# SmartBFT-Go/consensus

Hardware: NVIDIA H100
Metric: ECDSA-P256 verifies/sec at batch=64K (higher is better)
Workload: dtype u32 limbs (integer)

## Files before the change

### consensus_b200/csrc/inst_common.cuh

```cuda
#pragma once
#include "key_cache.cuh"
#include "keygroup.cuh"
#include "ops.h"

namespace sbv {

template <class C> struct Cfg;
template <> struct Cfg<P256> {
    static constexpr int COZ_MINB = 6, GPART_MINB = 6, KT_MINB = 6, COMB_MINB = 6;
    static constexpr bool KT_INL = true, COMB_INL = true;
};
template <> struct Cfg<P384> {
    static constexpr int COZ_MINB = 4, GPART_MINB = 3, KT_MINB = 4;
    static constexpr bool KT_INL = false;
};

template <class C>
cudaError_t op_gtable_init(uint32_t *gtab, cudaStream_t st) {
    const size_t entries = (size_t)C::GWINS << C::GW;
    k_gtable_init<C><<<(unsigned)((entries + 127) / 128), 128, 0, st>>>(gtab);
    return cudaGetLastError();
}

template <class C>
cudaError_t op_prep(uint32_t n, const uint8_t *r, const uint8_t *s, const uint8_t *dig, uint32_t dlen, uint32_t *uw, uint8_t *flags,
                    cudaStream_t st) {
    return launch_prep<C, 8>(n, r, s, dig, dlen, uw, flags, st);
}

template <class C>
cudaError_t op_group(uint32_t n, const uint8_t *qx, const uint8_t *qy, uint32_t seed, uint32_t hmask, uint32_t *htab, uint32_t *rep,
                     uint32_t *kcnt, uint32_t threshold, uint32_t max_keys, int32_t *keyid, uint32_t *keylist, uint32_t *counters,
                     cudaStream_t st) {
    const unsigned blocks = (n + 255) / 256;
    k_kg_insert<<<blocks, 256, 0, st>>>(n, KgXY<C>{qx, qy}, seed, hmask, htab, rep, kcnt);
    k_kg_assign<<<blocks, 256, 0, st>>>(n, rep, kcnt, threshold, max_keys, keyid, keylist, counters);
    return cudaGetLastError();
}

inline cudaError_t op_route(uint32_t n, const uint32_t *rep, const int32_t *keyid, int32_t *item_kid, uint32_t *klist, uint32_t *glist,
                            uint32_t *counters, cudaStream_t st) {
    k_kg_route<<<(n + 255) / 256, 256, 0, st>>>(n, rep, keyid, item_kid, klist, glist, counters);
    return cudaGetLastError();
}

template <class C>
cudaError_t op_gpart(uint32_t n, const uint32_t *uw, const uint32_t *gtab, uint32_t *gacc, cudaStream_t st) {
    constexpr int BLOCK = 64;
    k_gpart<C, BLOCK, Cfg<C>::GPART_MINB><<<(n + BLOCK - 1) / BLOCK, BLOCK, 0, st>>>(n, uw, reinterpret_cast<const uint4 *>(gtab), gacc);
    return cudaGetLastError();
}

template <class C>
cudaError_t op_coz(uint32_t n, const uint8_t *qx, const uint8_t *qy, const uint8_t *r, const uint32_t *uw, const uint8_t *flags,
                   const uint32_t *gtab, uint32_t *tscr, uint8_t *ok, const uint32_t *list, const uint32_t *count, cudaStream_t st) {
    constexpr int BLOCK = 64;
    const size_t smem = (size_t)7 * 2 * C::N * 4 * BLOCK;
    k_verify_coz<C, BLOCK, Cfg<C>::COZ_MINB><<<(n + BLOCK - 1) / BLOCK, BLOCK, smem, st>>>(
        n, qx, qy, r, uw, flags, reinterpret_cast<const uint4 *>(gtab), tscr, ok, list, count);
    return cudaGetLastError();
}

template <class C, int W>
cudaError_t op_kt_build(const uint32_t *nkeys_ptr, uint32_t cap, const uint32_t *keylist, const uint8_t *qx, const uint8_t *qy,
                        uint32_t *bases, uint32_t *hs, uint32_t *ztop, uint32_t *pref, uint32_t *ktab, uint8_t *keyflags, cudaStream_t st) {
    using KT = KeyTab<32 * C::N, W>;
    const unsigned kb = (cap + 63) / 64;
    const unsigned wb = (unsigned)(((size_t)cap * KT::NWIN + 63) / 64);
    k_kt_bases4<C, KT><<<(unsigned)(((size_t)cap * 4 + 127) / 128), 128, 0, st>>>(nkeys_ptr, cap, keylist, qx, qy, bases, keyflags);
    k_kt_fill<C, W><<<wb, 64, 0, st>>>(nkeys_ptr, cap, bases, keyflags, hs, ztop, ktab);
    k_kt_inv<C, KT><<<kb, 64, 0, st>>>(nkeys_ptr, cap, keyflags, ztop, pref);
    k_kt_final<C, KT><<<wb, 64, 0, st>>>(nkeys_ptr, cap, bases, keyflags, hs, ztop, ktab);
    return cudaGetLastError();
}

template <class C, int W>
cudaError_t op_kt_verify_grouped(uint32_t n, const int32_t *kidmap, const uint8_t *keyflags, const uint8_t *r, const uint32_t *uw, const uint8_t *flags,
                                 const uint32_t *gtab, const uint32_t *ktab, uint8_t *ok, const uint32_t *list, const uint32_t *count,
                                 const uint32_t *gacc, cudaStream_t st) {
    constexpr int BLOCK = 64;
    k_verify_kt<C, W, BLOCK, Cfg<C>::KT_MINB, false, Cfg<C>::KT_INL><<<(n + BLOCK - 1) / BLOCK, BLOCK, 0, st>>>(
        n, nullptr, kidmap, 0, keyflags, r, uw, flags, reinterpret_cast<const uint4 *>(gtab), reinterpret_cast<const uint4 *>(ktab), ok, list, count,
        gacc);
    return cudaGetLastError();
}

template <class C, int W>
cudaError_t op_kt_verify_registered(uint32_t n, const uint32_t *slot, const int32_t *slot2local, uint32_t n_slots, const uint8_t *keyflags,
                                    const uint8_t *r, const uint32_t *uw, const uint8_t *flags, const uint32_t *gtab, const uint32_t *ktab,
                                    uint8_t *ok, int warp, cudaStream_t st) {
    constexpr int BLOCK = 64;
    const uint4 *g4 = reinterpret_cast<const uint4 *>(gtab), *k4 = reinterpret_cast<const uint4 *>(ktab);
    if (warp)
        k_verify_kt_warp<C, W><<<(unsigned)(((size_t)n * 32 + 127) / 128), 128, 0, st>>>(n, slot, slot2local, n_slots, keyflags, r, uw, flags, g4, k4, ok);
    else
        k_verify_kt<C, W, BLOCK, Cfg<C>::KT_MINB, true, Cfg<C>::KT_INL><<<(n + BLOCK - 1) / BLOCK, BLOCK, 0, st>>>(
            n, slot, slot2local, n_slots, keyflags, r, uw, flags, g4, k4, ok, nullptr, nullptr, nullptr);
    return cudaGetLastError();
}

template <class C>
cudaError_t op_comb_build(const uint32_t *nkeys_ptr, uint32_t cap, const uint32_t *keylist, const uint8_t *qx, const uint8_t *qy,
                          uint32_t *bases, uint32_t *hs, uint32_t *ztop, uint32_t *pref, uint32_t *ktab, uint8_t *keyflags, cudaStream_t st) {
    using CT = CombTab<C>;
    const unsigned kb = (cap + 63) / 64;
    const unsigned cb = (unsigned)(((size_t)cap * CT::NCHAIN + 63) / 64);
    k_kt_bases4<C, CT><<<(unsigned)(((size_t)cap * 4 + 127) / 128), 128, 0, st>>>(nkeys_ptr, cap, keylist, qx, qy, bases, keyflags);
    k_comb_affine<C><<<kb, 64, 0, st>>>(nkeys_ptr, cap, keyflags, bases, pref);
    k_comb_fill<C><<<cb, 64, 0, st>>>(nkeys_ptr, cap, bases, keyflags, hs, ztop, ktab);
    k_kt_inv<C, CT><<<kb, 64, 0, st>>>(nkeys_ptr, cap, keyflags, ztop, pref);
    k_kt_final<C, CT><<<cb, 64, 0, st>>>(nkeys_ptr, cap, bases, keyflags, hs, ztop, ktab);
    return cudaGetLastError();
}

template <class C>
cudaError_t op_comb_verify(uint32_t n, const int32_t *kidmap, const uint8_t *keyflags, const uint8_t *r, const uint32_t *uw, const uint8_t *flags,
                           const uint32_t * , const uint32_t *ktab, uint8_t *ok, const uint32_t *list,
                           const uint32_t *count, const uint32_t *gacc, cudaStream_t st) {
    constexpr int BLOCK = 64;
    k_verify_comb<C, BLOCK, Cfg<C>::COMB_MINB, Cfg<C>::COMB_INL><<<(n + BLOCK - 1) / BLOCK, BLOCK, 0, st>>>(
        n, kidmap, keyflags, r, uw, flags, reinterpret_cast<const uint4 *>(ktab), ok, list, count, gacc);
    return cudaGetLastError();
}

template <class C>
cudaError_t op_kc_lookup(const uint32_t *nkeys_ptr, uint32_t kcap, const uint32_t *keylist, const uint8_t *qx, const uint8_t *qy, KcMap c, uint32_t tw4,
                         int32_t *keyid, uint32_t *lk, uint8_t *keyflags, uint32_t *ktab, cudaStream_t st) {
    k_kc_lookup<<<(unsigned)(((size_t)kcap * 32 + 127) / 128), 128, 0, st>>>(nkeys_ptr, kcap, keylist, KcXY<C>{qx, qy}, c, tw4, keyid, lk, keyflags,
                                                                            reinterpret_cast<uint4 *>(ktab));
    return cudaGetLastError();
}

template <class C>
cudaError_t op_kc_insert(uint32_t kcap, const uint32_t *lk, const uint8_t *qx, const uint8_t *qy, KcMap c, uint32_t tw4, const uint8_t *keyflags,
                         const uint32_t *ktab, cudaStream_t st) {
    k_kc_insert<<<(unsigned)(((size_t)kcap * 32 + 127) / 128), 128, 0, st>>>(kcap, lk, KcXY<C>{qx, qy}, c, tw4, keyflags,
                                                                            reinterpret_cast<const uint4 *>(ktab));
    return cudaGetLastError();
}

template <class C, class KT>
constexpr KtGeom kt_geom() {
    using KS = KtSizes<C, KT>;
    return KtGeom{KS::bases_words(1), KS::hs_words(1), KS::ztop_words(1), KS::ktab_words(1)};
}

}
```

### consensus_b200/csrc/keygroup.cuh

```cuda
#pragma once
#include "kernels.cuh"

namespace sbv {

constexpr uint32_t KG_EMPTY = 0xffffffffu;

SBV_DEV uint32_t kg_mix(uint32_t h, uint32_t w) {
    h = (h ^ w) * 0x9E3779B1u;
    h ^= h >> 15;
    return h * 0x85EBCA77u;
}
template <class C>
SBV_DEV uint32_t kg_hash(const uint8_t *__restrict__ qx_be, const uint8_t *__restrict__ qy_be, uint32_t i, uint32_t seed) {
    const uint32_t *x = reinterpret_cast<const uint32_t *>(qx_be + (size_t)i * C::BYTES);
    const uint32_t *y = reinterpret_cast<const uint32_t *>(qy_be + (size_t)i * C::BYTES);
    uint32_t h = seed;
#pragma unroll
    for (int k = 0; k < C::N; k++) {
        h = kg_mix(h, __ldg(x + k));
        h = kg_mix(h, __ldg(y + k));
    }
    return h ^ (h >> 16);
}
template <class C>
SBV_DEV bool kg_same_key(const uint8_t *__restrict__ qx_be, const uint8_t *__restrict__ qy_be, uint32_t i, uint32_t j) {
    const uint32_t *xi = reinterpret_cast<const uint32_t *>(qx_be + (size_t)i * C::BYTES);
    const uint32_t *xj = reinterpret_cast<const uint32_t *>(qx_be + (size_t)j * C::BYTES);
    const uint32_t *yi = reinterpret_cast<const uint32_t *>(qy_be + (size_t)i * C::BYTES);
    const uint32_t *yj = reinterpret_cast<const uint32_t *>(qy_be + (size_t)j * C::BYTES);
    uint32_t diff = 0;
#pragma unroll
    for (int k = 0; k < C::N; k++) diff |= (__ldg(xi + k) ^ __ldg(xj + k)) | (__ldg(yi + k) ^ __ldg(yj + k));
    return diff == 0;
}

template <class C>
struct KgXY {
    const uint8_t *qx_be, *qy_be;
    SBV_DEV uint32_t hash(uint32_t i, uint32_t seed) const { return kg_hash<C>(qx_be, qy_be, i, seed); }
    SBV_DEV bool same(uint32_t i, uint32_t j) const { return kg_same_key<C>(qx_be, qy_be, i, j); }
};
struct KgKey32 {
    const uint8_t *pub;
    SBV_DEV uint32_t hash(uint32_t i, uint32_t seed) const {
        const uint32_t *x = reinterpret_cast<const uint32_t *>(pub + (size_t)i * 32);
        uint32_t h = seed;
#pragma unroll
        for (int k = 0; k < 8; k += 2) {
            h = (h ^ __ldg(x + k)) * 0x9E3779B1u;
            h = (h ^ __ldg(x + k + 1)) * 0x85EBCA77u;
            h ^= h >> 15;
        }
        return h;
    }
    SBV_DEV bool same(uint32_t i, uint32_t j) const {
        const uint32_t *xi = reinterpret_cast<const uint32_t *>(pub + (size_t)i * 32);
        const uint32_t *xj = reinterpret_cast<const uint32_t *>(pub + (size_t)j * 32);
        uint32_t diff = 0;
#pragma unroll
        for (int k = 0; k < 8; k++) diff |= __ldg(xi + k) ^ __ldg(xj + k);
        return diff == 0;
    }
};

template <class KV>
__global__ void __launch_bounds__(256) k_kg_insert(uint32_t n, KV key, uint32_t seed, uint32_t hmask, uint32_t *__restrict__ htab,
                                                   uint32_t *__restrict__ rep, uint32_t *__restrict__ kcnt) {
    const uint32_t i = blockIdx.x * blockDim.x + threadIdx.x;
    if (i >= n) return;
    uint32_t h = key.hash(i, seed) & hmask;
    uint32_t r;
    for (;;) {
        uint32_t cur = htab[h];
        if (cur == KG_EMPTY) {
            cur = atomicCAS(htab + h, KG_EMPTY, i);
            if (cur == KG_EMPTY) { r = i; break; }
        }
        if (key.same(i, cur)) { r = cur; break; }
        h = (h + 1) & hmask;
    }
    rep[i] = r;
#if defined(__CUDA_ARCH__)
    const uint32_t peers = __match_any_sync(__activemask(), r);
    if ((threadIdx.x & 31) == (uint32_t)(__ffs((int)peers) - 1)) atomicAdd(kcnt + r, (uint32_t)__popc(peers));
#else
    atomicAdd(kcnt + r, 1u);
#endif
}

static __global__ void __launch_bounds__(256) k_kg_assign(uint32_t n, const uint32_t *__restrict__ rep, const uint32_t *__restrict__ kcnt,
                                                   uint32_t threshold, uint32_t max_keys, int32_t *__restrict__ keyid,
                                                   uint32_t *__restrict__ keylist, uint32_t *__restrict__ counters) {
    const uint32_t i = blockIdx.x * blockDim.x + threadIdx.x;
    if (i >= n) return;
    int32_t id = -1;
    if (rep[i] == i && kcnt[i] >= threshold) {
        const uint32_t k = atomicAdd(counters + 0, 1u);
        if (k < max_keys) { id = (int32_t)k; keylist[k] = i; }
    }
    keyid[i] = id;
}

static __global__ void __launch_bounds__(256) k_kg_route(uint32_t n, const uint32_t *__restrict__ rep, const int32_t *__restrict__ keyid,
                                                  int32_t *__restrict__ item_kid, uint32_t *__restrict__ klist, uint32_t *__restrict__ glist,
                                                  uint32_t *__restrict__ counters) {
    const uint32_t i = blockIdx.x * blockDim.x + threadIdx.x;
    const bool live = i < n;
    const int32_t kid = live ? keyid[rep[i]] : -1;
    if (live) item_kid[i] = kid;
#if defined(__CUDA_ARCH__)
    const uint32_t lane = threadIdx.x & 31;
    const uint32_t mk = __ballot_sync(0xffffffffu, live && kid >= 0), mg = __ballot_sync(0xffffffffu, live && kid < 0);
    uint32_t bk = 0, bg = 0;
    if (lane == 0) {
        if (mk) bk = atomicAdd(counters + 1, (uint32_t)__popc(mk));
        if (mg) bg = atomicAdd(counters + 2, (uint32_t)__popc(mg));
    }
    bk = __shfl_sync(0xffffffffu, bk, 0);
    bg = __shfl_sync(0xffffffffu, bg, 0);
    const uint32_t below = (1u << lane) - 1u;
    if (live && kid >= 0) klist[bk + __popc(mk & below)] = i;
    if (live && kid < 0) glist[bg + __popc(mg & below)] = i;
#else
    if (live && kid >= 0) klist[atomicAdd(counters + 1, 1u)] = i;
    if (live && kid < 0) glist[atomicAdd(counters + 2, 1u)] = i;
#endif
}


template <class C, class KT>
__global__ void __launch_bounds__(64) k_kt_bases(const uint32_t *__restrict__ nkeys_ptr, uint32_t cap, const uint32_t *__restrict__ keylist,
                                                 const uint8_t *__restrict__ qx_be, const uint8_t *__restrict__ qy_be,
                                                 uint32_t *__restrict__ bases, uint8_t *__restrict__ keyflags) {
    constexpr int N = C::N;
    const uint32_t k = blockIdx.x * blockDim.x + threadIdx.x;
    uint32_t nkeys = __ldg(nkeys_ptr);
    if (nkeys > cap) nkeys = cap;
    if (k >= nkeys) return;
    const uint32_t item = keylist ? keylist[k] : k;
    Jac<C> B;
    const bool good = load_key<C>(B.X, B.Y, qx_be, qy_be, item);
    keyflags[k] = good ? 1 : 0;
    if (!good) return;
    C::get_one(B.Z);
#pragma unroll 1
    for (int win = 0; win < KT::NBASE; win++) {
        if (win) {
#pragma unroll 1
            for (int d = 0; d < KT::STEP; d++) pt_double<C>(B);
        }
        uint32_t *o = bases + (size_t)win * 3 * N * cap + k;
#pragma unroll
        for (int i = 0; i < N; i++) { o[(size_t)i * cap] = B.X[i]; o[(size_t)(N + i) * cap] = B.Y[i]; o[(size_t)(2 * N + i) * cap] = B.Z[i]; }
    }
}

template <class C, class KT>
__global__ void __launch_bounds__(128) k_kt_bases4(const uint32_t *__restrict__ nkeys_ptr, uint32_t cap, const uint32_t *__restrict__ keylist,
                                                   const uint8_t *__restrict__ qx_be, const uint8_t *__restrict__ qy_be,
                                                   uint32_t *__restrict__ bases, uint8_t *__restrict__ keyflags) {
    constexpr int N = C::N;
    const uint32_t gt = blockIdx.x * blockDim.x + threadIdx.x;
    const uint32_t k = gt >> 2, role = gt & 3;
    uint32_t nkeys = __ldg(nkeys_ptr);
    if (nkeys > cap) nkeys = cap;
    if (k >= nkeys) return;
    const unsigned qbase = (threadIdx.x & 31) & ~3u, qmask = 0xFu << qbase;
    const uint32_t item = keylist ? keylist[k] : k;
    uint32_t X[N], Y[N], Z[N];
    const bool good = load_key<C>(X, Y, qx_be, qy_be, item);
    if (role == 0) keyflags[k] = good ? 1 : 0;
    if (!good) return;
    C::get_one(Z);
    auto bcast = [&](uint32_t (&v)[N], unsigned src) {
#pragma unroll
        for (int i = 0; i < N; i++) v[i] = __shfl_sync(qmask, v[i], qbase + src);
    };
#pragma unroll 1
    for (int win = 0; win < KT::NBASE; win++) {
        if (win) {
#pragma unroll 1
            for (int d = 0; d < KT::STEP; d++) {
                uint32_t s[N], a[N], b[N], r1[N], r2[N], r3[N], r4[N], t1[N], t2[N];
                C::fadd(s, Y, Y);
                mp_select<N>(a, role == 1 || role == 2, s, Z);
                mp_select<N>(b, role == 1, s, Z);
                C::fmul(r1, a, b);
                uint32_t bb[N];
                mp_copy<N>(bb, r1);
                bcast(bb, 1);
                C::fsub(t1, X, r1);
                C::fadd(t2, X, r1);
                mp_select<N>(a, role == 0, t1, X);
                mp_select<N>(a, role == 2, bb, a);
                mp_select<N>(b, role == 0, t2, bb);
                C::fmul(r2, a, b);
                uint32_t alpha[N], half[N], beta4[N];
                C::fadd(t1, r2, r2);
                C::fadd(alpha, t1, r2);
                C::fhalf(half, r2);
                C::fmul(r3, alpha, alpha);
                mp_copy<N>(beta4, r2);
                bcast(beta4, 1);
                bcast(half, 2);
                uint32_t x3[N], y3[N];
                C::fadd(t1, beta4, beta4);
                C::fsub(x3, r3, t1);
                C::fsub(t2, beta4, x3);
                C::fmul(r4, alpha, t2);
                C::fsub(y3, r4, half);
                mp_copy<N>(X, x3); bcast(X, 0);
                mp_copy<N>(Y, y3); bcast(Y, 0);
                mp_copy<N>(Z, r1); bcast(Z, 2);
            }
        }
        if (role == 0) {
            uint32_t *o = bases + (size_t)win * 3 * N * cap + k;
#pragma unroll
            for (int i = 0; i < N; i++) { o[(size_t)i * cap] = X[i]; o[(size_t)(N + i) * cap] = Y[i]; o[(size_t)(2 * N + i) * cap] = Z[i]; }
        }
    }
}

template <class C>
SBV_DEV void zaddu(uint32_t (&X1)[C::N], uint32_t (&Y1)[C::N], const uint32_t (&X2)[C::N], const uint32_t (&Y2)[C::N],
                   uint32_t (&X3)[C::N], uint32_t (&Y3)[C::N], uint32_t (&h)[C::N]) {
    constexpr int N = C::N;
    uint32_t c[N], w1[N], w2[N], dy[N], d[N], a1[N], t[N];
    C::fsub(h, X1, X2);
    C::fsqr(c, h);
    C::fmul(w1, X1, c);
    C::fmul(w2, X2, c);
    C::fsub(dy, Y1, Y2);
    C::fsqr(d, dy);
    C::fsub(t, w1, w2);
    C::fmul(a1, Y1, t);
    C::fsub(X3, d, w1);
    C::fsub(X3, X3, w2);
    C::fsub(t, w1, X3);
    C::fmul(Y3, dy, t);
    C::fsub(Y3, Y3, a1);
    mp_copy<N>(X1, w1);
    mp_copy<N>(Y1, a1);
}

template <class C, int W>
__global__ void __launch_bounds__(64) k_kt_fill(const uint32_t *__restrict__ nkeys_ptr, uint32_t cap, const uint32_t *__restrict__ bases,
                                                const uint8_t *__restrict__ keyflags, uint32_t *__restrict__ hs,
                                                uint32_t *__restrict__ ztop, uint32_t *__restrict__ ktab) {
    constexpr int N = C::N;
    using KT = KeyTab<32 * N, W>;
    const uint32_t t = blockIdx.x * blockDim.x + threadIdx.x;
    uint32_t nkeys = __ldg(nkeys_ptr);
    if (nkeys > cap) nkeys = cap;
    if (t >= nkeys * KT::NWIN) return;
    const uint32_t k = t % nkeys, win = t / nkeys;
    if (!keyflags[k]) return;
    uint32_t bx[N], by[N], bz[N];
    {
        const uint32_t *o = bases + (size_t)win * 3 * N * cap + k;
#pragma unroll
        for (int i = 0; i < N; i++) { bx[i] = o[(size_t)i * cap]; by[i] = o[(size_t)(N + i) * cap]; bz[i] = o[(size_t)(2 * N + i) * cap]; }
    }
    uint32_t *out = ktab + ((size_t)k * KT::NWIN + win) * KT::ENT * 2 * N;
#pragma unroll
    for (int i = 0; i < N; i++) { out[i] = bx[i]; out[N + i] = by[i]; }
    Jac<C> P;
    mp_copy<N>(P.X, bx); mp_copy<N>(P.Y, by); mp_copy<N>(P.Z, bz);
    uint32_t h[N], h2[N], h3[N];
    C::fadd(h, by, by);
    pt_double<C>(P);
    C::fsqr(h2, h);
    C::fmul(h3, h2, h);
    C::fmul(bx, bx, h2);
    C::fmul(by, by, h3);
    uint32_t zacc[N];
    mp_copy<N>(zacc, P.Z);
    {
        uint32_t *hp = hs + ((size_t)win * (KT::ENT - 1) + 0) * N * cap + k;
#pragma unroll
        for (int i = 0; i < N; i++) { out[2 * N + i] = P.X[i]; out[3 * N + i] = P.Y[i]; hp[(size_t)i * cap] = h[i]; }
    }
    uint32_t px[N], py[N];
    mp_copy<N>(px, P.X); mp_copy<N>(py, P.Y);
#pragma unroll 1
    for (int e = 3; e <= KT::ENT; e++) {
        uint32_t x3[N], y3[N];
        zaddu<C>(bx, by, px, py, x3, y3, h);
        C::fmul(zacc, zacc, h);
        mp_copy<N>(px, x3); mp_copy<N>(py, y3);
        uint32_t *hp = hs + ((size_t)win * (KT::ENT - 1) + (e - 2)) * N * cap + k;
        uint32_t *oe = out + (size_t)(e - 1) * 2 * N;
#pragma unroll
        for (int i = 0; i < N; i++) { oe[i] = px[i]; oe[N + i] = py[i]; hp[(size_t)i * cap] = h[i]; }
    }
    uint32_t *zp = ztop + (size_t)win * N * cap + k;
#pragma unroll
    for (int i = 0; i < N; i++) zp[(size_t)i * cap] = zacc[i];
}

template <class C, class KT>
__global__ void __launch_bounds__(64) k_kt_inv(const uint32_t *__restrict__ nkeys_ptr, uint32_t cap, const uint8_t *__restrict__ keyflags,
                                               uint32_t *__restrict__ ztop, uint32_t *__restrict__ pref) {
    constexpr int N = C::N;
    const uint32_t k = blockIdx.x * blockDim.x + threadIdx.x;
    uint32_t nkeys = __ldg(nkeys_ptr);
    if (nkeys > cap) nkeys = cap;
    if (k >= nkeys || !keyflags[k]) return;
    uint32_t run[N];
    C::get_one(run);
#pragma unroll 1
    for (int win = 0; win < KT::NCHAIN; win++) {
        uint32_t z[N];
        const uint32_t *zp = ztop + (size_t)win * N * cap + k;
        uint32_t *pp = pref + (size_t)win * N * cap + k;
#pragma unroll
        for (int i = 0; i < N; i++) { z[i] = zp[(size_t)i * cap]; pp[(size_t)i * cap] = run[i]; }
        C::fmul(run, run, z);
    }
    uint32_t inv[N];
    p_inv<C>(inv, run);
#pragma unroll 1
    for (int win = KT::NCHAIN - 1; win >= 0; win--) {
        uint32_t z[N], pv[N], zi[N];
        uint32_t *zp = ztop + (size_t)win * N * cap + k;
        const uint32_t *pp = pref + (size_t)win * N * cap + k;
#pragma unroll
        for (int i = 0; i < N; i++) { z[i] = zp[(size_t)i * cap]; pv[i] = pp[(size_t)i * cap]; }
        C::fmul(zi, inv, pv);
        C::fmul(inv, inv, z);
#pragma unroll
        for (int i = 0; i < N; i++) zp[(size_t)i * cap] = zi[i];
    }
}

template <class C, class KT>
__global__ void __launch_bounds__(64) k_kt_final(const uint32_t *__restrict__ nkeys_ptr, uint32_t cap, const uint32_t *__restrict__ bases,
                                                 const uint8_t *__restrict__ keyflags, const uint32_t *__restrict__ hs,
                                                 const uint32_t *__restrict__ ztop, uint32_t *__restrict__ ktab) {
    constexpr int N = C::N;
    const uint32_t t = blockIdx.x * blockDim.x + threadIdx.x;
    uint32_t nkeys = __ldg(nkeys_ptr);
    if (nkeys > cap) nkeys = cap;
    if (t >= nkeys * KT::NCHAIN) return;
    const uint32_t k = t % nkeys, win = t / nkeys;
    if (!keyflags[k]) return;
    uint32_t zi[N];
    {
        const uint32_t *zp = ztop + (size_t)win * N * cap + k;
#pragma unroll
        for (int i = 0; i < N; i++) zi[i] = zp[(size_t)i * cap];
    }
    uint32_t *out = ktab + ((size_t)k * KT::NCHAIN + win) * KT::ENT * 2 * N;
    uint32_t x[N], y[N], h[N];
    {
        const uint32_t *oe = out + (size_t)(KT::ENT - 1) * 2 * N;
#pragma unroll
        for (int i = 0; i < N; i++) { x[i] = oe[i]; y[i] = oe[N + i]; }
    }
#pragma unroll 1
    for (int e = KT::ENT; e >= 1; e--) {
        uint32_t nx[N], ny[N], nh[N];
        if (e >= 2) {
            const uint32_t *on = out + (size_t)(e - 2) * 2 * N;
            const uint32_t *hp = hs + ((size_t)win * (KT::ENT - 1) + (e - 2)) * N * cap + k;
#pragma unroll
            for (int i = 0; i < N; i++) { nx[i] = on[i]; ny[i] = on[N + i]; nh[i] = hp[(size_t)i * cap]; }
        }
        uint32_t *oe = out + (size_t)(e - 1) * 2 * N;
        uint32_t z2[N], z3[N];
        C::fsqr(z2, zi);
        C::fmul(z3, z2, zi);
        C::fmul(x, x, z2);
        C::fmul(y, y, z3);
#pragma unroll
        for (int i = 0; i < N; i++) { oe[i] = x[i]; oe[N + i] = y[i]; }
        if (e >= 2) {
            mp_copy<N>(h, nh);
            C::fmul(zi, zi, h);
            mp_copy<N>(x, nx); mp_copy<N>(y, ny);
        }
    }
    (void)bases;
}


template <class C>
__global__ void __launch_bounds__(64) k_comb_affine(const uint32_t *__restrict__ nkeys_ptr, uint32_t cap, const uint8_t *__restrict__ keyflags,
                                                    uint32_t *__restrict__ bases, uint32_t *__restrict__ pref) {
    constexpr int N = C::N;
    using CT = CombTab<C>;
    const uint32_t k = blockIdx.x * blockDim.x + threadIdx.x;
    uint32_t nkeys = __ldg(nkeys_ptr);
    if (nkeys > cap) nkeys = cap;
    if (k >= nkeys || !keyflags[k]) return;
    uint32_t run[N];
    C::get_one(run);
#pragma unroll 1
    for (int c = 0; c < CT::NBASE; c++) {
        uint32_t z[N];
        const uint32_t *zp = bases + ((size_t)c * 3 + 2) * N * cap + k;
        uint32_t *pp = pref + (size_t)c * N * cap + k;
#pragma unroll
        for (int i = 0; i < N; i++) { z[i] = zp[(size_t)i * cap]; pp[(size_t)i * cap] = run[i]; }
        C::fmul(run, run, z);
    }
    uint32_t inv[N];
    p_inv<C>(inv, run);
#pragma unroll 1
    for (int c = CT::NBASE - 1; c >= 0; c--) {
        uint32_t *o = bases + (size_t)c * 3 * N * cap + k;
        const uint32_t *pp = pref + (size_t)c * N * cap + k;
        uint32_t x[N], y[N], z[N], pv[N], zi[N], z2[N], z3[N];
#pragma unroll
        for (int i = 0; i < N; i++) { x[i] = o[(size_t)i * cap]; y[i] = o[(size_t)(N + i) * cap]; z[i] = o[(size_t)(2 * N + i) * cap]; pv[i] = pp[(size_t)i * cap]; }
        C::fmul(zi, inv, pv);
        C::fmul(inv, inv, z);
        C::fsqr(z2, zi);
        C::fmul(z3, z2, zi);
        C::fmul(x, x, z2);
        C::fmul(y, y, z3);
#pragma unroll
        for (int i = 0; i < N; i++) { o[(size_t)i * cap] = x[i]; o[(size_t)(N + i) * cap] = y[i]; }
    }
}

template <class C>
__global__ void __launch_bounds__(64) k_comb_fill(const uint32_t *__restrict__ nkeys_ptr, uint32_t cap, const uint32_t *__restrict__ bases,
                                                  const uint8_t *__restrict__ keyflags, uint32_t *__restrict__ hs,
                                                  uint32_t *__restrict__ ztop, uint32_t *__restrict__ ktab) {
    constexpr int N = C::N;
    using CT = CombTab<C>;
    const uint32_t t = blockIdx.x * blockDim.x + threadIdx.x;
    uint32_t nkeys = __ldg(nkeys_ptr);
    if (nkeys > cap) nkeys = cap;
    if (t >= nkeys * CT::NCHAIN) return;
    const uint32_t k = t % nkeys, ch = t / nkeys;
    if (!keyflags[k]) return;
    const int b = (int)(ch >> 4), hi = (int)(ch & 15);
    auto base = [&](int c, uint32_t (&x)[N], uint32_t (&y)[N]) {
        const uint32_t *o = bases + (size_t)c * 3 * N * cap + k;
#pragma unroll
        for (int i = 0; i < N; i++) { x[i] = o[(size_t)i * cap]; y[i] = o[(size_t)(N + i) * cap]; }
    };
    uint32_t *out = ktab + ((size_t)k * CT::NCHAIN + ch) * CT::ENT * 2 * N;
    auto store = [&](int slot, const uint32_t (&x)[N], const uint32_t (&y)[N], const uint32_t (&h)[N]) {
        uint32_t *o = out + (size_t)slot * 2 * N;
#pragma unroll
        for (int i = 0; i < N; i++) { o[i] = x[i]; o[N + i] = y[i]; }
        if (slot) {
            uint32_t *hp = hs + ((size_t)ch * (CT::ENT - 1) + (slot - 1)) * N * cap + k;
#pragma unroll
            for (int i = 0; i < N; i++) hp[(size_t)i * cap] = h[i];
        }
    };
    Jac<C> P;
    uint32_t x[N], y[N], h[N];
    C::get_one(P.Z);
    C::get_one(h);
    int first;
    if (hi == 0) {
        uint32_t zero[N];
#pragma unroll
        for (int i = 0; i < N; i++) zero[i] = 0;
        store(0, zero, zero, h);
        base(CT::TEETH * b, P.X, P.Y);
        store(1, P.X, P.Y, h);
        first = 2;
    } else {
        bool empty = true;
#pragma unroll 1
        for (int i = 0; i < 4; i++) {
            if (!((hi >> i) & 1)) continue;
            base(CT::TEETH * b + 4 + i, x, y);
            if (empty) { mp_copy<N>(P.X, x); mp_copy<N>(P.Y, y); empty = false; }
            else pt_madd_table<C>(P, x, y, h);
        }
        store(0, P.X, P.Y, h);
        first = 1;
    }
#pragma unroll 1
    for (int kk = first; kk < CT::ENT; kk++) {
        const int tooth = __ffs(kk) - 1;
        base(CT::TEETH * b + tooth, x, y);
        if (!(((kk ^ (kk >> 1)) >> tooth) & 1)) {
            uint32_t zero[N];
#pragma unroll
            for (int i = 0; i < N; i++) zero[i] = 0;
            C::fsub(y, zero, y);
        }
        pt_madd_table<C>(P, x, y, h);
        store(kk, P.X, P.Y, h);
    }
    uint32_t *zp = ztop + (size_t)ch * N * cap + k;
#pragma unroll
    for (int i = 0; i < N; i++) zp[(size_t)i * cap] = P.Z[i];
}

template <class C, class KT_>
struct KtSizes {
    using KT = KT_;
    static constexpr size_t bases_words(size_t cap) { return (size_t)KT::NBASE * 3 * C::N * cap; }
    static constexpr size_t hs_words(size_t cap) { return (size_t)KT::NCHAIN * (KT::ENT - 1) * C::N * cap; }
    static constexpr size_t ztop_words(size_t cap) { return (size_t)KT::NCHAIN * C::N * cap; }
    static constexpr size_t ktab_words(size_t cap) { return KT::POINTS * 2 * C::N * cap; }
};

}
```

Baseline: 66.54 million.

## Split comb base doubling across thread pairs and inline arithmetic in table build

```diff
diff --git a/consensus_b200/csrc/inst_common.cuh b/consensus_b200/csrc/inst_common.cuh
--- a/consensus_b200/csrc/inst_common.cuh
+++ b/consensus_b200/csrc/inst_common.cuh
@@ -105,11 +105,12 @@
     using CT = CombTab<C>;
     const unsigned kb = (cap + 63) / 64;
     const unsigned cb = (unsigned)(((size_t)cap * CT::NCHAIN + 63) / 64);
-    k_kt_bases4<C, CT><<<(unsigned)(((size_t)cap * 4 + 127) / 128), 128, 0, st>>>(nkeys_ptr, cap, keylist, qx, qy, bases, keyflags);
+    constexpr bool INL = Cfg<C>::COMB_INL;
+    k_kt_bases2<C, CT, INL><<<(unsigned)(((size_t)cap * 2 + 127) / 128), 128, 0, st>>>(nkeys_ptr, cap, keylist, qx, qy, bases, keyflags);
     k_comb_affine<C><<<kb, 64, 0, st>>>(nkeys_ptr, cap, keyflags, bases, pref);
-    k_comb_fill<C><<<cb, 64, 0, st>>>(nkeys_ptr, cap, bases, keyflags, hs, ztop, ktab);
+    k_comb_fill<C, INL><<<cb, 64, 0, st>>>(nkeys_ptr, cap, bases, keyflags, hs, ztop, ktab);
     k_kt_inv<C, CT><<<kb, 64, 0, st>>>(nkeys_ptr, cap, keyflags, ztop, pref);
-    k_kt_final<C, CT><<<cb, 64, 0, st>>>(nkeys_ptr, cap, bases, keyflags, hs, ztop, ktab);
+    k_kt_final<C, CT, INL><<<cb, 64, 0, st>>>(nkeys_ptr, cap, bases, keyflags, hs, ztop, ktab);
     return cudaGetLastError();
 }
 
diff --git a/consensus_b200/csrc/keygroup.cuh b/consensus_b200/csrc/keygroup.cuh
--- a/consensus_b200/csrc/keygroup.cuh
+++ b/consensus_b200/csrc/keygroup.cuh
@@ -222,6 +222,100 @@
     }
 }
 
+template <class C, class KT, bool INL>
+__global__ void __launch_bounds__(128) k_kt_bases2(const uint32_t *__restrict__ nkeys_ptr, uint32_t cap, const uint32_t *__restrict__ keylist,
+                                                   const uint8_t *__restrict__ qx_be, const uint8_t *__restrict__ qy_be,
+                                                   uint32_t *__restrict__ bases, uint8_t *__restrict__ keyflags) {
+    using A = typename PickArith<C, INL>::type;
+    constexpr int N = C::N;
+    const uint32_t gt = blockIdx.x * blockDim.x + threadIdx.x;
+    const uint32_t k = gt >> 1, role = gt & 1;
+    uint32_t nkeys = __ldg(nkeys_ptr);
+    if (nkeys > cap) nkeys = cap;
+    if (k >= nkeys) return;
+    const unsigned pbase = (threadIdx.x & 31) & ~1u, pmask = 3u << pbase, other = pbase + (role ^ 1);
+    const uint32_t item = keylist ? keylist[k] : k;
+    uint32_t X[N], Y[N], Z[N];
+    const bool good = load_key<C>(X, Y, qx_be, qy_be, item);
+    if (role == 0) keyflags[k] = good ? 1 : 0;
+    if (!good) return;
+    C::get_one(Z);
+    auto xchg = [&](uint32_t (&v)[N]) {
+#pragma unroll
+        for (int i = 0; i < N; i++) v[i] = __shfl_sync(pmask, v[i], other);
+    };
+#pragma unroll 1
+    for (int win = 0; win < KT::NBASE; win++) {
+        if (win) {
+#pragma unroll 1
+            for (int d = 0; d < KT::STEP; d++) {
+                uint32_t s[N], a[N], b[N], r1[N], r2[N], r3[N], r4[N], t1[N], t2[N];
+                C::fadd(s, Y, Y);
+                mp_select<N>(a, role == 1, s, Z);
+                A::fsqr(r1, a);
+                C::fsub(t1, X, r1);
+                C::fadd(t2, X, r1);
+                mp_select<N>(a, role == 1, X, t1);
+                mp_select<N>(b, role == 1, r1, t2);
+                A::fmul(r2, a, b);
+                uint32_t beta4[N], alpha[N];
+                mp_copy<N>(beta4, r2);
+                xchg(beta4);
+                C::fadd(t1, r2, r2);
+                C::fadd(alpha, t1, r2);
+                mp_select<N>(a, role == 1, r1, alpha);
+                A::fsqr(r3, a);
+                uint32_t x3[N], c8[N];
+                C::fadd(t1, beta4, beta4);
+                C::fsub(t2, r3, t1);
+                C::fhalf(t1, r3);
+                mp_select<N>(x3, role == 1, t1, t2);
+                xchg(x3);
+                mp_select<N>(c8, role == 1, t1, x3);
+                mp_select<N>(x3, role == 1, x3, t2);
+                C::fsub(t1, beta4, x3);
+                mp_select<N>(a, role == 1, s, alpha);
+                mp_select<N>(b, role == 1, Z, t1);
+                A::fmul(r4, a, b);
+                C::fsub(t2, r4, c8);
+                mp_select<N>(t1, role == 1, r4, t2);
+                xchg(t1);
+                mp_copy<N>(X, x3);
+                mp_select<N>(Y, role == 1, t1, t2);
+                mp_select<N>(Z, role == 1, r4, t1);
+            }
+        }
+        if (role == 0) {
+            uint32_t *o = bases + (size_t)win * 3 * N * cap + k;
+#pragma unroll
+            for (int i = 0; i < N; i++) { o[(size_t)i * cap] = X[i]; o[(size_t)(N + i) * cap] = Y[i]; o[(size_t)(2 * N + i) * cap] = Z[i]; }
+        }
+    }
+}
+
+template <int N>
+SBV_DEV void st_entry(uint32_t *o, const uint32_t (&x)[N], const uint32_t (&y)[N]) {
+    uint4 *v = reinterpret_cast<uint4 *>(o);
+#pragma unroll
+    for (int i = 0; i < N / 4; i++) {
+        uint4 a, b;
+        a.x = x[4 * i]; a.y = x[4 * i + 1]; a.z = x[4 * i + 2]; a.w = x[4 * i + 3];
+        b.x = y[4 * i]; b.y = y[4 * i + 1]; b.z = y[4 * i + 2]; b.w = y[4 * i + 3];
+        v[i] = a;
+        v[N / 4 + i] = b;
+    }
+}
+template <int N>
+SBV_DEV void ld_entry(const uint32_t *o, uint32_t (&x)[N], uint32_t (&y)[N]) {
+    const uint4 *v = reinterpret_cast<const uint4 *>(o);
+#pragma unroll
+    for (int i = 0; i < N / 4; i++) {
+        const uint4 a = v[i], b = v[N / 4 + i];
+        x[4 * i] = a.x; x[4 * i + 1] = a.y; x[4 * i + 2] = a.z; x[4 * i + 3] = a.w;
+        y[4 * i] = b.x; y[4 * i + 1] = b.y; y[4 * i + 2] = b.z; y[4 * i + 3] = b.w;
+    }
+}
+
 template <class C>
 SBV_DEV void zaddu(uint32_t (&X1)[C::N], uint32_t (&Y1)[C::N], const uint32_t (&X2)[C::N], const uint32_t (&Y2)[C::N],
                    uint32_t (&X3)[C::N], uint32_t (&Y3)[C::N], uint32_t (&h)[C::N]) {
@@ -334,10 +428,11 @@
     }
 }
 
-template <class C, class KT>
+template <class C, class KT, bool INL = false>
 __global__ void __launch_bounds__(64) k_kt_final(const uint32_t *__restrict__ nkeys_ptr, uint32_t cap, const uint32_t *__restrict__ bases,
                                                  const uint8_t *__restrict__ keyflags, const uint32_t *__restrict__ hs,
                                                  const uint32_t *__restrict__ ztop, uint32_t *__restrict__ ktab) {
+    using A = typename PickArith<C, INL>::type;
     constexpr int N = C::N;
     const uint32_t t = blockIdx.x * blockDim.x + threadIdx.x;
     uint32_t nkeys = __ldg(nkeys_ptr);
@@ -354,30 +449,26 @@
     uint32_t *out = ktab + ((size_t)k * KT::NCHAIN + win) * KT::ENT * 2 * N;
     uint32_t x[N], y[N], h[N];
     {
-        const uint32_t *oe = out + (size_t)(KT::ENT - 1) * 2 * N;
-#pragma unroll
-        for (int i = 0; i < N; i++) { x[i] = oe[i]; y[i] = oe[N + i]; }
+        ld_entry<N>(out + (size_t)(KT::ENT - 1) * 2 * N, x, y);
     }
 #pragma unroll 1
     for (int e = KT::ENT; e >= 1; e--) {
         uint32_t nx[N], ny[N], nh[N];
         if (e >= 2) {
-            const uint32_t *on = out + (size_t)(e - 2) * 2 * N;
             const uint32_t *hp = hs + ((size_t)win * (KT::ENT - 1) + (e - 2)) * N * cap + k;
-#pragma unroll
-            for (int i = 0; i < N; i++) { nx[i] = on[i]; ny[i] = on[N + i]; nh[i] = hp[(size_t)i * cap]; }
-        }
-        uint32_t *oe = out + (size_t)(e - 1) * 2 * N;
+            ld_entry<N>(out + (size_t)(e - 2) * 2 * N, nx, ny);
+#pragma unroll
+            for (int i = 0; i < N; i++) nh[i] = hp[(size_t)i * cap];
+        }
         uint32_t z2[N], z3[N];
-        C::fsqr(z2, zi);
-        C::fmul(z3, z2, zi);
-        C::fmul(x, x, z2);
-        C::fmul(y, y, z3);
-#pragma unroll
-        for (int i = 0; i < N; i++) { oe[i] = x[i]; oe[N + i] = y[i]; }
+        A::fsqr(z2, zi);
+        A::fmul(z3, z2, zi);
+        A::fmul(x, x, z2);
+        A::fmul(y, y, z3);
+        st_entry<N>(out + (size_t)(e - 1) * 2 * N, x, y);
         if (e >= 2) {
             mp_copy<N>(h, nh);
-            C::fmul(zi, zi, h);
+            A::fmul(zi, zi, h);
             mp_copy<N>(x, nx); mp_copy<N>(y, ny);
         }
     }
@@ -425,10 +516,11 @@
     }
 }
 
-template <class C>
+template <class C, bool INL>
 __global__ void __launch_bounds__(64) k_comb_fill(const uint32_t *__restrict__ nkeys_ptr, uint32_t cap, const uint32_t *__restrict__ bases,
                                                   const uint8_t *__restrict__ keyflags, uint32_t *__restrict__ hs,
                                                   uint32_t *__restrict__ ztop, uint32_t *__restrict__ ktab) {
+    using A = typename PickArith<C, INL>::type;
     constexpr int N = C::N;
     using CT = CombTab<C>;
     const uint32_t t = blockIdx.x * blockDim.x + threadIdx.x;
@@ -445,52 +537,39 @@
     };
     uint32_t *out = ktab + ((size_t)k * CT::NCHAIN + ch) * CT::ENT * 2 * N;
     auto store = [&](int slot, const uint32_t (&x)[N], const uint32_t (&y)[N], const uint32_t (&h)[N]) {
-        uint32_t *o = out + (size_t)slot * 2 * N;
-#pragma unroll
-        for (int i = 0; i < N; i++) { o[i] = x[i]; o[N + i] = y[i]; }
+        st_entry<N>(out + (size_t)slot * 2 * N, x, y);
         if (slot) {
             uint32_t *hp = hs + ((size_t)ch * (CT::ENT - 1) + (slot - 1)) * N * cap + k;
 #pragma unroll
             for (int i = 0; i < N; i++) hp[(size_t)i * cap] = h[i];
         }
     };
-    Jac<C> P;
-    uint32_t x[N], y[N], h[N];
+    Jac<A> P;
+    uint32_t x[N], y[N], h[N], zero[N];
+#pragma unroll
+    for (int i = 0; i < N; i++) zero[i] = 0;
     C::get_one(P.Z);
     C::get_one(h);
-    int first;
-    if (hi == 0) {
-        uint32_t zero[N];
-#pragma unroll
-        for (int i = 0; i < N; i++) zero[i] = 0;
-        store(0, zero, zero, h);
-        base(CT::TEETH * b, P.X, P.Y);
-        store(1, P.X, P.Y, h);
-        first = 2;
-    } else {
-        bool empty = true;
-#pragma unroll 1
-        for (int i = 0; i < 4; i++) {
-            if (!((hi >> i) & 1)) continue;
-            base(CT::TEETH * b + 4 + i, x, y);
-            if (empty) { mp_copy<N>(P.X, x); mp_copy<N>(P.Y, y); empty = false; }
-            else pt_madd_table<C>(P, x, y, h);
-        }
-        store(0, P.X, P.Y, h);
-        first = 1;
-    }
-#pragma unroll 1
-    for (int kk = first; kk < CT::ENT; kk++) {
-        const int tooth = __ffs(kk) - 1;
+    if (hi == 0) store(0, zero, zero, h);
+    const int nhigh = __popc(hi);
+    int rest = hi;
+#pragma unroll 1
+    for (int st = 0; st < nhigh + CT::ENT - 1; st++) {
+        const int kk = st - nhigh + 1;
+        int tooth;
+        bool sub = false;
+        if (kk <= 0) {
+            tooth = 4 + __ffs(rest) - 1;
+            rest &= rest - 1;
+        } else {
+            tooth = __ffs(kk) - 1;
+            sub = !(((kk ^ (kk >> 1)) >> tooth) & 1);
+        }
         base(CT::TEETH * b + tooth, x, y);
-        if (!(((kk ^ (kk >> 1)) >> tooth) & 1)) {
-            uint32_t zero[N];
-#pragma unroll
-            for (int i = 0; i < N; i++) zero[i] = 0;
-            C::fsub(y, zero, y);
-        }
-        pt_madd_table<C>(P, x, y, h);
-        store(kk, P.X, P.Y, h);
+        if (sub) C::fsub(y, zero, y);
+        if (st == 0) { mp_copy<N>(P.X, x); mp_copy<N>(P.Y, y); }
+        else pt_madd_table<A>(P, x, y, h);
+        if (kk >= 0) store(kk, P.X, P.Y, h);
     }
     uint32_t *zp = ztop + (size_t)ch * N * cap + k;
 #pragma unroll
```

New measurement: 70.66 million, median of 6. 1.06x the previous value.
